# mrmod/h264decode

Measured on AMD Instinct MI355X. Metric: 1080p Main CABAC frames/sec, higher is better.
Workload: dtype u8; 1 GPU; 1920x1080 Main CABAC IPPP GOP-30, 256 independent streams per GPU (32 distinct, each used 8 times), QP 28, 1 slice/frame, 1 ref; parallelism=streams sharded, no collective

## Files before the change

h264decode_amd/csrc/k_entropy.hip:

```cpp
#include <hip/hip_runtime.h>
#include "mi_kernels.h"

#ifndef MI_ENT_ISLICE_PRIO
#define MI_ENT_ISLICE_PRIO 0
#endif
#ifndef MI_ENT_MINWAVES
#define MI_ENT_MINWAVES 6
#endif
#ifndef MI_ENT_B
#define MI_ENT_B 0
#endif
#ifndef MI_ENT_FMO
#define MI_ENT_FMO MI_ENT_B
#endif
#if MI_ENT_B
#define NL 2
#define MI_ENT_KERNEL k_entropy_b
#elif MI_ENT_FMO
#define NL 1
#define MI_ENT_KERNEL k_entropy_f
#else
#define NL 1
#define MI_ENT_KERNEL k_entropy
#endif
#define LANE (e.lane)
#define FI __device__ __forceinline__
#define LDS_SYNC()                                             \
    do {                                                       \
        __builtin_amdgcn_fence(__ATOMIC_RELEASE, "wavefront"); \
        __builtin_amdgcn_wave_barrier();                       \
        __builtin_amdgcn_fence(__ATOMIC_ACQUIRE, "wavefront"); \
    } while (0)

struct TopInfo {
    uint8_t type, t8x8, cbp, chroma_mode, cbf_dc;
    uint8_t dmask;
    uint16_t row;
// ... 728 lines not shown
            off = NB_TL * TB, k = 3;
        else if (gy < 0 && gx == 4)
            off = (NB_TOP + 1) * TB, k = 0, tr = 1;
        const uint32_t interior = gx >= 0 && gx < 4 && gy >= 0;
        return off | k << 9 | edge << 11 | interior << 12 | tr << 13;
    }
    if (l >= 32 && l < 50) {
        const int i = l - 32, cpl = i / 9, g = i % 9, gx = g % 3 - 1, gy = g / 3 - 1;
        uint32_t off = NO_SRC, left = 0;
        if (gy < 0 && gx >= 0)
            off = NB_TOP * TB + static_cast<uint32_t>(offsetof(TopInfo, nnz)) + 4 + cpl * 2 + gx;
        else if (gx < 0 && gy >= 0)
            off = NB_LEFT * TB + static_cast<uint32_t>(offsetof(TopInfo, nnz)) + 4 + cpl * 2 + gy, left = 1;
        const uint32_t interior = gx >= 0 && gy >= 0;
        return off | interior << 12 | left << 14 | static_cast<uint32_t>(cpl * 12 + g) << 16;
    }
    if (l >= 50 && l < 56) {
        const uint32_t left = l < 53;
        return ((left ? NB_LEFT : NB_TOP) * TB + static_cast<uint32_t>(offsetof(TopInfo, cbf_dc))) | static_cast<uint32_t>((l - 50) % 3) << 9 | left << 14;
    }
    return NO_SRC;
}

FI void fill_caches(Ent &e) {
    Shared *s = e.s;
    const bool a_ok = (e.aw & 255) != 0, b_ok = (e.bw & 255) != 0;
    const int cip = e.cip;
    int l = LANE;
    OPAQUE(l);
    const uint32_t role = s->role[l], off = role & NO_SRC;
    const uint8_t *nbb = reinterpret_cast<const uint8_t *>(s->nb);
    int coded = 0;
    if (l < 30) {
        int8_t ipm = -2;
        uint8_t nnz = 0x80;
        const int k = static_cast<int>((role >> 9) & 3u);
        const bool has = off != NO_SRC && !((role >> 13) & 1u && e.mbx + 1 >= e.wmb);
        const TopInfo *n = reinterpret_cast<const TopInfo *>(nbb + (off != NO_SRC ? off : 0u));
        const bool n_ok = has && n->type != MBT_NONE;
        if (n_ok) {
            const int inter = MB_IS_INTER(n->type);
            if (!(cip && inter)) ipm = (n->type == MBT_I4x4 || n->type == MBT_I8x8) ? n->ipm[k] : static_cast<int8_t>(2);
            if ((role >> 11) & 1u) nnz = n->nnz[k];
        }
#pragma unroll
        for (int L = 0; L < NL; L++) {
            int8_t ref = -2, refi = -2;
            uint8_t mvdx = 0, mvdy = 0;
            int16_t mvx = 0, mvy = 0;
            if (n_ok) {
                if (MB_IS_INTER(n->type)) {
                    ref = refi = n->ref[L][k >> 1];
                    mvx = n->mv[L][k][0], mvy = n->mv[L][k][1];
                    mvdx = n->mvd[L][k][0], mvdy = n->mvd[L][k][1];
                    if (MI_ENT_B && ((n->dmask >> (k >> 1)) & 1)) refi = 0;
                } else
                    ref = refi = -1;
            }
            s->ref_c[L][l] = ref;
            s->refi_c[L][l] = refi;
            s->mv_c[L][l][0] = mvx, s->mv_c[L][l][1] = mvy;
            s->mvd_c[L][l][0] = mvdx, s->mvd_c[L][l][1] = mvdy;
        }
        if ((role >> 12) & 1u) {
            nnz = 0;
            ipm = -1;
        }
        coded = (nnz & 0x80) ? 2 : (nnz != 0);
        s->ipm_c[l] = ipm;
        e.v_ipm = ipm;
        s->nnz_c[l] = nnz;
    } else if (l >= 32 && l < 50) {
        const bool ok = off != NO_SRC && (((role >> 14) & 1u) ? a_ok : b_ok);
        const uint8_t v = ((role >> 12) & 1u) ? static_cast<uint8_t>(0) : (ok ? nbb[off != NO_SRC ? off : 0u] : static_cast<uint8_t>(0x80));
        coded = (v & 0x80) ? 2 : (v != 0);
        (&s->nnzc_c[0][0])[(role >> 16) & 31u] = v;
    } else if (l >= 50 && l < 56) {
        const bool ok = ((role >> 14) & 1u) ? a_ok : b_ok;
        coded = ok ? (nbb[off] >> ((role >> 9) & 3u)) & 1 : 2;
    } else if (l >= 56) {
        s->refs8[(l - 56) >> 2][l & 3] = -1;
        if (l < 60) s->sub_type[l - 56] = 0;
        if (l == 60) s->cur_cbf_dc = 0;
    }
    s->coded[l] = static_cast<uint8_t>(coded);
    LDS_SYNC();
}

#if MI_ENT_B
FI int min_positive(int a, int b) { return (a >= 0 && b >= 0) ? min(a, b) : max(a, b); }
FI int b_pair_modes(int k) { return static_cast<int>((0xFB7ED69A5ull >> (4 * k)) & 15); }
FI int b_sub_mode(int st) { return static_cast<int>((0x39FA5E4u >> (2 * st)) & 3); }
FI int b_sub_shape(int st) { return static_cast<int>((0x3F99900u >> (2 * st)) & 3); }
static_assert(((0x39FA5E4u >> 8) & 3) == 1 && ((0x39FA5E4u >> 24) & 3) == 3 && ((0x39FA5E4u >> 12) & 3) == 2 && ((0x3F99900u >> 8) & 3) == 1 && ((0x3F99900u >> 10) & 3) == 2,
              "Table 7-18 constants");

FI void direct_pred(Ent &e, int mask8, bool commit) {
    Shared *s = e.s;
    int l = LANE;
    OPAQUE(l);
    if (l < 20) s->col[l] = e.v_col;
    LDS_SYNC();
    const int bx = l & 3, by = (l >> 2) & 3, q = (by >> 1) * 2 + (bx >> 1);
    const int cb = e.d8inf ? (by >> 1) * 12 + (bx >> 1) * 3 : (l & 15);
// ... 48 lines not shown
        }
        if (!((bx | by) & 1)) {
            if (commit)
                s->refs8[0][q] = static_cast<int8_t>(ref0), s->refs8[1][q] = static_cast<int8_t>(ref1);
            else
                s->dref[0][q] = static_cast<int8_t>(ref0), s->dref[1][q] = static_cast<int8_t>(ref1);
        }
    }
    LDS_SYNC();
}
FI void commit_direct(Ent &e, const int L, int q) {
    Shared *s = e.s;
    const int l = LANE, bx = l & 3, by = (l >> 2) & 3;
    if (l < 16 && (by >> 1) * 2 + (bx >> 1) == q) {
        const int g = GI(bx, by);
        s->ref_c[L][g] = s->dref[L][q];
        *reinterpret_cast<uint32_t *>(s->mv_c[L][g]) = *reinterpret_cast<const uint32_t *>(s->dmv[L][l]);
        if (!((bx | by) & 1)) s->refs8[L][q] = s->dref[L][q];
    }
    LDS_SYNC();
}
#endif

FI void read_ref_idx(Ent &e, const int L, int bx, int by, int w, int h, int nref) {
    Shared *s = e.s;
    int ref = 0;
    if (nref > 1) {
        if (e.cabac) {
            int ctx = (s->refi_c[L][GI(bx - 1, by)] > 0) + 2 * (s->refi_c[L][GI(bx, by - 1)] > 0);
            while (BIN_A(e, 54 + ctx)) {
                ctx = (ctx >> 2) + 4;
                if (++ref > 31) {
                    e.err = 3;
                    break;
                }
            }
        } else
            ref = nref == 2 ? !get_bit(e) : static_cast<int>(get_ue(e));
        if (ref >= nref || ref >= MI_MAX_REFS) e.err = 13, ref = 0;
    }
    {
        const int l = LANE, x = l & 3, y = (l >> 2) & 3;
        if (l < 16 && x >= bx && x < bx + w && y >= by && y < by + h) {
            s->refi_c[L][GI(x, y)] = static_cast<int8_t>(ref);
            if (!((x | y) & 1)) s->refs8[L][(y >> 1) * 2 + (x >> 1)] = static_cast<int8_t>(ref);
        }
        LDS_SYNC();
    }
}
FI void read_mv(Ent &e, const int L, int p) {
    Shared *s = e.s;
    const int bx = p & 3, by = (p >> 2) & 3, w = ((p >> 4) & 3) + 1, h = ((p >> 6) & 3) + 1, shape = (p >> 8) & 7;
    const int ref = s->refs8[L][(by >> 1) * 2 + (bx >> 1)];
    int d[2];
    for (int comp = 0; comp < 2; comp++) {
        int v;
        if (e.cabac) {
            const int sum = s->mvd_c[L][GI(bx - 1, by)][comp] + s->mvd_c[L][GI(bx, by - 1)][comp];
            const int base = comp ? 47 : 40;
            v = 0;
            if (BIN_A(e, base + (sum > 2) + (sum > 32))) {
                int ctx = base + 3;
                v = 1;
                while (v < 9 && BIN_A(e, ctx)) {
                    if (v < 4) ctx++;
                    v++;
                }
                if (v >= 9) v += cabac_egk(e, 3);
                if (cabac_bypass(e)) v = -v;
            }
        } else
            v = get_se(e);
        d[comp] = v;
    }
    int px, py;
    predict_mv(e, L, bx, by, w, ref, shape, px, py);
    set_part(e, L, bx, by, w, h, ref, px + d[0], py + d[1], d[0], d[1]);
}

#if !MI_ENT_B
FI void pskip_fast(Ent &e) {
    Shared *s = e.s;
    int l = LANE;
    OPAQUE(l);
    const uint32_t *nbw = reinterpret_cast<const uint32_t *>(s->nb);
    const uint32_t tA = e.aw, tB = e.bw, tC = nbw[(NB_TOP + 1) * TOP_DW], tD = nbw[NB_TL * TOP_DW];
    const uint32_t rA = nbw[NB_LEFT * TOP_DW + 5], rB = nbw[NB_TOP * TOP_DW + 5], rC = nbw[(NB_TOP + 1) * TOP_DW + 5], rD = nbw[NB_TL * TOP_DW + 5];
    const uint32_t mA = nbw[NB_LEFT * TOP_DW + 6], mB = nbw[NB_TOP * TOP_DW + 6], mC = nbw[(NB_TOP + 1) * TOP_DW + 6], mD = nbw[NB_TL * TOP_DW + 9];
    auto ref_of = [](uint32_t t, uint32_t r, int byte) {
        const int type = static_cast<int>(t & 255u);
        return type == MBT_NONE ? -2 : (MB_IS_INTER(type) ? static_cast<int>(static_cast<int8_t>((r >> (8 * byte)) & 255u)) : -1);
    };
    auto mv_of = [](uint32_t t, uint32_t m) { return MB_IS_INTER(static_cast<int>(t & 255u)) ? m : 0u; };
    const int ra = ref_of(tA, rA, 0), rb = ref_of(tB, rB, 0);
    const bool c_ok = e.mbx + 1 < e.wmb && (tC & 255u) != MBT_NONE;
    const int rc = c_ok ? ref_of(tC, rC, 0) : ref_of(tD, rD, 1);
    const uint32_t va = mv_of(tA, mA), vb = mv_of(tB, mB), vc = c_ok ? mv_of(tC, mC) : mv_of(tD, mD);
    uint32_t mvw = 0;
    const bool zero = ra == -2 || rb == -2 || (ra == 0 && va == 0) || (rb == 0 && vb == 0);
    if (!zero) {
        const int na = ra == 0, nb_ = rb == 0, nc = rc == 0;
        if (na + nb_ + nc == 1)
            mvw = na ? va : (nb_ ? vb : vc);
        else {
            const int ax = static_cast<int16_t>(va & 0xffffu), ay = static_cast<int32_t>(va) >> 16, bx = static_cast<int16_t>(vb & 0xffffu), by = static_cast<int32_t>(vb) >> 16;
            const int cx = static_cast<int16_t>(vc & 0xffffu), cy = static_cast<int32_t>(vc) >> 16;
            mvw = (static_cast<uint32_t>(median3(ax, bx, cx)) & 0xffffu) | (static_cast<uint32_t>(median3(ay, by, cy)) << 16);
        }
    }
    e.cur_type = MBT_PSKIP;
    e.prev_dqp_nz = 0;
    if (l < TOP_DW) {
        const uint32_t row = MI_ENT_FMO ? static_cast<uint32_t>(e.mby + 1) << 16 : 0u;
        const uint32_t nw = l == 0 ? static_cast<uint32_t>(MBT_PSKIP) : (l == 1 ? row : (l == 2 ? 0xFFFFFFFFu : ((l >= 6 && l < 10) ? mvw : 0u)));
        uint32_t *tl = reinterpret_cast<uint32_t *>(&s->nb[NB_TL]), *tp = reinterpret_cast<uint32_t *>(&s->nb[NB_TOP]), *tr = reinterpret_cast<uint32_t *>(&s->nb[NB_TOP + 1]);
        const uint32_t old_top = tp[l], w1 = tr[l];
        tl[l] = old_top;
        tp[l] = w1;
        tr[l] = e.pre_top;
        reinterpret_cast<uint32_t *>(&s->nb[NB_LEFT])[l] = nw;
        reinterpret_cast<uint32_t *>(e.top + e.mbx)[l] = nw;
        e.pre_top = top_load(e, e.mbx + 3, l);
    } else if (l >= 32) {
        const int k = l - 32;
        const uint32_t t = s->skip_tmpl[k];
        const uint32_t w = k == 0 ? (static_cast<uint32_t>(MBT_PSKIP) | e.qpw0) : (k == 1 ? e.qpw1 : ((k >= 12 && k < 28) ? mvw : t));
        const uint64_t mbi = e.mb_base + static_cast<uint64_t>(e.mby) * e.wmb + e.mbx;
        reinterpret_cast<uint32_t *>(e.mbrec + mbi)[k] = w;
    }
    LDS_SYNC();
}
#endif

FI void decode_mb(Ent &e, int skipped) {
    Shared *s = e.s;
    MbRec &r = s->rec;
    const int cabac = e.cabac, islice = e.islice;
    int cbp_luma = 0, cbp_chroma = 0, t8x8 = 0, i16mode = 0, chroma_mode = 0, has_coef = 0;
    int type, raw = 0, nparts = 0;
    const Nb a{e.aw}, b{e.bw};
    r.nzmask = 0;
#if MI_ENT_B
    int no_sub8 = 1;
    e.direct8 = 0;
#endif
    if (skipped) {
#if MI_ENT_B
        type = MBT_BSKIP;
        e.cur_type = type;
        e.direct8 = 15;
        direct_pred(e, 15, true);
#else
        type = MBT_PSKIP;
        e.cur_type = type;
        int mvx = 0, mvy = 0;
        int ra = s->ref_c[0][GI(-1, 0)], rb = s->ref_c[0][GI(0, -1)];
        bool zero = ra == -2 || rb == -2 || (ra == 0 && s->mv_c[0][GI(-1, 0)][0] == 0 && s->mv_c[0][GI(-1, 0)][1] == 0) ||
                    (rb == 0 && s->mv_c[0][GI(0, -1)][0] == 0 && s->mv_c[0][GI(0, -1)][1] == 0);
        if (!zero) predict_mv(e, 0, 0, 0, 4, 0, 0, mvx, mvy);
        set_part(e, 0, 0, 0, 4, 4, 0, mvx, mvy, 0, 0);
        s->refs8[0][0] = s->refs8[0][1] = s->refs8[0][2] = s->refs8[0][3] = 0;
#endif
        e.prev_dqp_nz = 0;
// ... 8 lines not shown
                if (!BIN_A(e, 27 + inc))
                    raw = 0;
                else if (!BIN_A(e, 27 + 3))
                    raw = 1 + BINI_A(e, 27 + 5);
                else {
                    int bits = BINI_A(e, 27 + 4) << 3;
                    bits |= BINI_A(e, 27 + 5) << 2;
                    bits |= BINI_A(e, 27 + 5) << 1;
                    bits |= BINI_A(e, 27 + 5);
                    if (bits < 8)
                        raw = bits + 3;
                    else if (bits == 13)
                        intra_prefix = 1;
                    else if (bits == 14)
                        raw = 11;
                    else if (bits == 15)
                        raw = 22;
                    else
                        raw = ((bits << 1) | BINI_A(e, 27 + 5)) - 4;
                }
            }
#else
            if (!islice) {
                intra_prefix = BINI_A(e, 14);
                if (!intra_prefix) raw = BIN_A(e, 15) ? 2 - BINI_A(e, 17) : 3 * BINI_A(e, 16);
            }
#endif
            if (intra_prefix) {
                int base = islice ? 3 : (MI_ENT_B ? 32 : 17), it = 0, first;
                if (islice) {
                    int inc = (a.ok() && a.type() != MBT_I4x4 && a.type() != MBT_I8x8) + (b.ok() && b.type() != MBT_I4x4 && b.type() != MBT_I8x8);
                    first = BINI_A(e, base + inc);
                    base += 2;
                } else
                    first = BINI_A(e, base);
                if (first) {
                    if (cabac_terminate(e))
                        it = 25;
                    else {
                        it = 1 + 12 * BINI_A(e, base + 1);
                        if (BIN_A(e, base + 2)) it += 4 + 4 * BINI_A(e, base + 2 + islice);
                        it += 2 * BINI_A(e, base + 3 + islice);
                        it += BINI_A(e, base + 3 + 2 * islice);
                    }
                }
                raw = islice ? it : it + (MI_ENT_B ? 23 : 5);
            }
        } else
            raw = static_cast<int>(get_ue(e));
        const int it = islice ? raw : raw - (MI_ENT_B ? 23 : 5);
#if MI_ENT_B
        if (raw < 23)
            type = raw == 0 ? MBT_BDIRECT : MBT_B;
#else
        if (!islice && raw < 5)
            type = raw == 0 ? MBT_P16x16 : (raw == 1 ? MBT_P16x8 : (raw == 2 ? MBT_P8x16 : MBT_P8x8));
#endif
        else if (it == 0)
            type = MBT_I4x4;
        else if (it >= 1 && it <= 24) {
            type = MBT_I16x16;
            i16mode = (it - 1) & 3;
            cbp_chroma = ((it - 1) >> 2) % 3;
            cbp_luma = it >= 13 ? 15 : 0;
            if (cbp_chroma && e.mono) e.err = 25, cbp_chroma = 0;
        } else if (it == 25)
// ... 88 lines not shown
                            int bx, by, w, h, md;
                            if (raw == 22)
                                bx = (i & 1) * 2, by = (i >> 1) * 2, w = 2, h = 2, md = b_sub_mode(s->sub_type[i]);
                            else {
                                const int p = s->parts[i];
                                bx = p & 3, by = (p >> 2) & 3, w = ((p >> 4) & 3) + 1, h = ((p >> 6) & 3) + 1, md = p >> 11;
                            }
                            if ((md >> L) & 1) read_ref_idx(e, L, bx, by, w, h, L ? e.nref1 : e.nref);
                        }
#pragma unroll
                    for (int L = 0; L < 2; L++)
                        for (int i = 0; i < nparts; i++) {
                            const int p = s->parts[i], md = p >> 11;
                            const int bx = p & 3, by = (p >> 2) & 3;
                            if (md == 0)
                                commit_direct(e, L, (by >> 1) * 2 + (bx >> 1));
                            else if ((md >> L) & 1)
                                read_mv(e, L, p);
                            else
                                set_part(e, L, bx, by, ((p >> 4) & 3) + 1, ((p >> 6) & 3) + 1, -1, 0, 0, 0, 0);
                        }
                }
#else
                int nref_parts;
                if (type == MBT_P16x16) {
                    s->parts[0] = PART(0, 0, 4, 4, 0);
                    nparts = nref_parts = 1;
                } else if (type == MBT_P16x8) {
                    s->parts[0] = PART(0, 0, 4, 2, 1), s->parts[1] = PART(0, 2, 4, 2, 2);
                    nparts = nref_parts = 2;
                } else if (type == MBT_P8x16) {
                    s->parts[0] = PART(0, 0, 2, 4, 3), s->parts[1] = PART(2, 0, 2, 4, 4);
                    nparts = nref_parts = 2;
                } else {
                    nref_parts = 4;
                    for (int i = 0; i < 4; i++) {
                        int st;
                        if (cabac)
                            st = BIN_A(e, 21) ? 0 : (!BIN_A(e, 22) ? 1 : (BIN_A(e, 23) ? 2 : 3));
                        else
                            st = static_cast<int>(get_ue(e));
                        if (st > 3) e.err = 21, st = 0;
                        s->sub_type[i] = static_cast<int8_t>(st);
                        const int bx = (i & 1) * 2, by = (i >> 1) * 2;
                        const int sw = (st == 0 || st == 1) ? 2 : 1, sh = (st == 0 || st == 2) ? 2 : 1;
                        for (int yy = 0; yy < 2; yy += sh)
                            for (int xx = 0; xx < 2; xx += sw) s->parts[nparts++] = PART(bx + xx, by + yy, sw, sh, 0);
                    }
                }
                for (int i = 0; i < nref_parts; i++) {
                    int bx, by, w, h;
                    if (type == MBT_P8x8)
                        bx = (i & 1) * 2, by = (i >> 1) * 2, w = 2, h = 2;
                    else {
                        const int p = s->parts[i];
                        bx = p & 3, by = (p >> 2) & 3, w = ((p >> 4) & 3) + 1, h = ((p >> 6) & 3) + 1;
                    }
                    read_ref_idx(e, 0, bx, by, w, h, raw != 4 ? e.nref : 1);
                }
                for (int i = 0; i < nparts; i++) read_mv(e, 0, s->parts[i]);
#endif
            } else {
                if (type == MBT_I4x4 && e.t8x8_mode) {
                    t8x8 = cabac ? BINI_T8(e, (a.ok() && a.t8x8()) + (b.ok() && b.t8x8())) : static_cast<int>(get_bit(e));
                    if (t8x8) type = MBT_I8x8, e.cur_type = type;
                }
                if (type == MBT_I4x4 || type == MBT_I8x8) {
                    const int n = type == MBT_I8x8 ? 4 : 16;
                    for (int i = 0; i < n; i++) {
                        int bx, by;
                        if (n == 4)
                            bx = (i & 1) * 2, by = (i >> 1) * 2;
                        else
                            bx = (i & 1) + 2 * ((i >> 2) & 1), by = ((i >> 1) & 1) + 2 * (i >> 3);
                        const int pa = static_cast<int>(RDL(e.v_ipm, GI(bx - 1, by))), pb = static_cast<int>(RDL(e.v_ipm, GI(bx, by - 1)));
                        const int pred = (pa < -1 || pb < -1) ? 2 : (pa < pb ? pa : pb);
                        int mode = pred;
                        if (cabac) {
                            if (!BIN_B(e, 68)) {
                                int rem = 0;
                                for (int k = 0; k < 3; k++) rem |= BINI_B(e, 69) << k;
                                mode = rem < pred ? rem : rem + 1;
                            }
// ... 8 lines not shown
                }
                if (e.mono)
                    chroma_mode = 0;
                else if (cabac) {
                    int inc = (a.ok() && MB_IS_INTRA(a.type()) && a.type() != MBT_IPCM && a.chroma_mode() != 0) +
                              (b.ok() && MB_IS_INTRA(b.type()) && b.type() != MBT_IPCM && b.chroma_mode() != 0);
                    chroma_mode = 0;
                    if (BIN_B(e, 64 + inc)) {
                        chroma_mode = 1;
                        while (chroma_mode < 3 && BIN_B(e, 67)) chroma_mode++;
                    }
                } else {
                    chroma_mode = static_cast<int>(get_ue(e));
                    if (chroma_mode > 3) e.err = 22, chroma_mode = 0;
                }
                if (LANE < 16) {
                    s->ref_c[0][GI(LANE & 3, LANE >> 2)] = -1;
                    if (MI_ENT_B) s->ref_c[NL - 1][GI(LANE & 3, LANE >> 2)] = -1;
                }
            }
            MI_S(e, MB_IS_INTER(type) ? 1 : 2);
            if (type != MBT_I16x16) {
                int cbp;
                if (cabac) {
                    const int cbp_a = a.ok() ? (a.type() == MBT_IPCM ? 0x2F : a.cbp()) : 0x0F;
                    const int cbp_b = b.ok() ? (b.type() == MBT_IPCM ? 0x2F : b.cbp()) : 0x0F;
                    cbp = 0;
                    for (int b8 = 0; b8 < 4; b8++) {
                        int ca = (b8 & 1) ? (cbp >> (b8 - 1)) & 1 : (cbp_a >> (b8 + 1)) & 1;
                        int cb = (b8 & 2) ? (cbp >> (b8 - 2)) & 1 : (cbp_b >> (b8 + 2)) & 1;
                        cbp |= BINI_B(e, 73 + (!ca) + 2 * (!cb)) << b8;
                    }
                    int ca = a.ok() && (a.type() == MBT_IPCM || (a.cbp() >> 4) != 0), cb = b.ok() && (b.type() == MBT_IPCM || (b.cbp() >> 4) != 0);
                    if (!e.mono && BIN_B(e, 77 + ca + 2 * cb)) {
                        ca = a.ok() && (a.type() == MBT_IPCM || (a.cbp() >> 4) == 2);
                        cb = b.ok() && (b.type() == MBT_IPCM || (b.cbp() >> 4) == 2);
                        cbp |= (1 + BINI_B(e, 77 + 4 + ca + 2 * cb)) << 4;
                    }
                } else {
                    uint32_t k = get_ue(e);
                    if (k > (e.mono ? 15u : 47u)) e.err = 23, k = 0;
                    if (e.mono) k += 48;
                    cbp = RFL(static_cast<int>(MB_IS_INTRA(type) ? e.tab->me_intra[k] : e.tab->me_inter[k]));
                }
                cbp_luma = cbp & 15, cbp_chroma = cbp >> 4;
                if (cbp_luma && e.t8x8_mode && MB_IS_INTER(type)) {
#if MI_ENT_B
                    const int all8 = no_sub8;
#else
                    int all8 = 1;
                    if (type == MBT_P8x8)
                        for (int i = 0; i < 4; i++) all8 &= s->sub_type[i] == 0;
#endif
                    if (all8) t8x8 = cabac ? BINI_T8(e, (a.ok() && a.t8x8()) + (b.ok() && b.t8x8())) : static_cast<int>(get_bit(e));
                }
            }
            if (cbp_luma || cbp_chroma || type == MBT_I16x16) {
                int dqp;
                if (cabac) {
                    int ctx = e.prev_dqp_nz ? 1 : 0, val = 0;
                    while (BIN_A(e, 60 + ctx)) {
                        ctx = 2 + (ctx >> 1);
// ... 93 lines not shown
    TopInfo *tp = &s->nb[NB_TOP];
    if (l >= 32 && l < 32 + TOP_DW) reinterpret_cast<uint32_t *>(&s->nb[NB_TL])[l - 32] = reinterpret_cast<const uint32_t *>(tp)[l - 32];
    LDS_SYNC();
    if (l < 2) {
        TopInfo *dst = &s->nb[l == 0 ? NB_TOP : NB_LEFT];
        dst->type = static_cast<uint8_t>(type);
        dst->t8x8 = static_cast<uint8_t>(t8x8);
        dst->cbp = r.cbp;
        dst->chroma_mode = static_cast<uint8_t>(chroma_mode);
        dst->cbf_dc = s->cur_cbf_dc;
        if (MI_ENT_FMO) dst->row = static_cast<uint16_t>(e.mby + 1);
#pragma unroll
        for (int L = 0; L < NL; L++) {
            dst->ref[L][0] = inter ? s->refs8[L][l == 0 ? 2 : 1] : static_cast<int8_t>(-1);
            dst->ref[L][1] = inter ? s->refs8[L][3] : static_cast<int8_t>(-1);
        }
#if MI_ENT_B
        dst->dmask = static_cast<uint8_t>(l == 0 ? (e.direct8 >> 2) & 3 : ((e.direct8 >> 1) & 1) | ((e.direct8 >> 2) & 2));
#endif
    } else if (l >= 8 && l < 16) {
        int k = l & 3, is_left = l >= 12;
        TopInfo *dst = &s->nb[is_left ? NB_LEFT : NB_TOP];
        int g = is_left ? GI(3, k) : GI(k, 3);
        dst->ipm[k] = s->ipm_c[g];
        dst->nnz[k] = s->nnz_c[g];
#pragma unroll
        for (int L = 0; L < NL; L++) {
            dst->mv[L][k][0] = s->mv_c[L][g][0], dst->mv[L][k][1] = s->mv_c[L][g][1];
            dst->mvd[L][k][0] = s->mvd_c[L][g][0], dst->mvd[L][k][1] = s->mvd_c[L][g][1];
        }
    } else if (l >= 16 && l < 24) {
        int i = l - 16, is_left = i >= 4, cpl = (i >> 1) & 1, k = i & 1;
        TopInfo *dst = &s->nb[is_left ? NB_LEFT : NB_TOP];
        dst->nnz[4 + cpl * 2 + k] = is_left ? s->nnzc_c[cpl][(k + 1) * 3 + 2] : s->nnzc_c[cpl][2 * 3 + k + 1];
    }
    LDS_SYNC();
    if (l < TOP_DW) {
        const uint32_t nw = reinterpret_cast<const uint32_t *>(tp)[l], w1 = reinterpret_cast<const uint32_t *>(&s->nb[NB_TOP + 1])[l];
        reinterpret_cast<uint32_t *>(e.top + e.mbx)[l] = nw;
        reinterpret_cast<uint32_t *>(&s->nb[NB_TOP])[l] = w1;
        reinterpret_cast<uint32_t *>(&s->nb[NB_TOP + 1])[l] = e.pre_top;
        e.pre_top = top_load(e, e.mbx + 3, l);
    }
    const uint64_t mbi = e.mb_base + static_cast<uint64_t>(e.mby) * e.wmb + e.mbx;
    if (l >= 32)
        reinterpret_cast<uint32_t *>(e.mbrec + mbi)[l - 32] = reinterpret_cast<const uint32_t *>(&r)[l - 32];
#if MI_ENT_B
// ... 138 lines not shown
    int addr = RFL(static_cast<int>(sd->first_mb));
    const bool fmo = MI_ENT_FMO && RFL(static_cast<int>(pd->fmo)) != 0;
    bool consecutive = false;
    if (!fmo) fill_none(e, RFL(static_cast<int>(sd->fill_from)), min(addr, total));
    e.mbx = addr % e.wmb, e.mby = addr / e.wmb;
    int more = 1, skip_state = 0 , pending = 0;
    int n_mbs = 0;
    while (more && !e.err) {
        if (addr >= total) {
            e.err = 30;
            break;
        }
        if (fmo) {
            asm volatile("s_waitcnt vmcnt(0)" ::: "memory");
            if (!consecutive && l < TOP_DW) {
                reinterpret_cast<uint32_t *>(&sh.nb[NB_LEFT])[l] = 0;
                reinterpret_cast<uint32_t *>(&sh.nb[NB_TL])[l] = e.mbx > 0 ? top_load(e, e.mbx - 1, l) : 0u;
            }
            if (l < 2 * TOP_DW) reinterpret_cast<uint32_t *>(&sh.nb[NB_TOP])[l] = top_load(e, e.mbx + l / TOP_DW, l % TOP_DW);
            LDS_SYNC();
            if (l < 3 && sh.nb[NB_TL + l].row != static_cast<uint16_t>(e.mby)) sh.nb[NB_TL + l].type = MBT_NONE;
            LDS_SYNC();
        } else if (e.mbx == 0 || n_mbs == 0) {
            if (l < TOP_DW) reinterpret_cast<uint32_t *>(&sh.nb[NB_LEFT])[l] = 0, reinterpret_cast<uint32_t *>(&sh.nb[NB_TL])[l] = 0;
            asm volatile("s_waitcnt vmcnt(0)" ::: "memory");
            if (l < 2 * TOP_DW) reinterpret_cast<uint32_t *>(&sh.nb[NB_TOP])[l] = top_load(e, e.mbx + l / TOP_DW, l % TOP_DW);
            if (l < TOP_DW) e.pre_top = top_load(e, e.mbx + 2, l);
            LDS_SYNC();
        }
        OPAQUE(e.lane);
        slide_window(e);
        MI_T0(e);
#if MI_ENT_B
        e.v_col = (e.col && l < 20) ? e.col[static_cast<size_t>(addr) * 20 + l] : ((l >= 16 && l < 19) ? 0xFFFFFFFFu : 0u);
#endif
        e.aw = RFL(*reinterpret_cast<const uint32_t *>(&sh.nb[NB_LEFT])), e.bw = RFL(*reinterpret_cast<const uint32_t *>(&sh.nb[NB_TOP]));
        int skipped = 0;
        if (!e.islice) {
            if (e.cabac) {
                const Nb a{e.aw}, b{e.bw};
                const int skip_type = MI_ENT_B ? MBT_BSKIP : MBT_PSKIP;
                skipped = BINI_A(e, (MI_ENT_B ? 24 : 11) + (a.ok() && a.type() != skip_type) + (b.ok() && b.type() != skip_type));
            } else {
                if (skip_state == 0) {
                    pending = static_cast<int>(get_ue(e));
                    if (pending > total - addr) e.err = 31, pending = 0;
                    if (pending > 0) skip_state = 1;
                }
                if (skip_state == 1) {
                    skipped = 1;
                    pending--;
                }
            }
        }
#if !MI_ENT_B
        if (skipped) {
            MI_T(e, 1);
            pskip_fast(e);
        } else
#endif
        {
            MI_T(e, 1);
            fill_caches(e);
            MI_T(e, 0);
            decode_mb(e, skipped);
        }
        MI_T(e, 3);
        if (e.err) break;
        n_mbs++;
        if (e.cabac)
            more = !cabac_terminate(e);
        else if (skipped) {
            if (pending == 0) {
                more = bitpos(e) < stop_bit;
                skip_state = 2;
            }
        } else {
            more = bitpos(e) < stop_bit;
            skip_state = 0;
        }
        if (fmo) {
            const uint8_t *sgmap = bitstream + RFL(e.pd->sgmap_off);
            const int sgroup = RFL(static_cast<int>(sgmap[RFL(static_cast<int>(e.sd->first_mb))]));
            const uint32_t inv_wmb = RFL(e.pd->inv_wmb);
            int next = total;
            for (int base = addr + 1; base < total; base += 64) {
                const int i = base + l;
                const unsigned long long m = __builtin_amdgcn_ballot_w64(i < total && sgmap[i] == sgroup);
                if (m) {
// ... 27 lines not shown
```

Before: 29380 frames/s.

## Add fast path for CABAC P16x16 macroblocks in entropy kernel

For non-B CABAC P slices, the mb_type prefix is now decoded before the neighbour caches are filled. P16x16 macroblocks decode ref_idx, mvd and cbp straight from packed neighbour words. A P16x16 with zero cbp leaves through a shared skip-style writer, which skips fill_caches and the general partition loops. A coded P16x16 runs a reduced fill_caches that omits ipm and per-block ref/mv setup. This is meant to cut LDS traffic and wave barriers per inter macroblock, at the cost of more code paths that must stay bit-exact.

```diff
diff --git a/h264decode_amd/csrc/k_entropy.hip b/h264decode_amd/csrc/k_entropy.hip
--- a/h264decode_amd/csrc/k_entropy.hip
+++ b/h264decode_amd/csrc/k_entropy.hip
@@ -13,6 +13,10 @@
 #ifndef MI_ENT_FMO
 #define MI_ENT_FMO MI_ENT_B
 #endif
+#ifndef MI_ENT_P16_DIRECT
+#define MI_ENT_P16_DIRECT 1
+#endif
+#define MI_P16 (MI_ENT_P16_DIRECT && !MI_ENT_B)
 #if MI_ENT_B
 #define NL 2
 #define MI_ENT_KERNEL k_entropy_b
@@ -787,7 +791,7 @@
     return NO_SRC;
 }
 
-FI void fill_caches(Ent &e) {
+FI void fill_caches(Ent &e, bool p16 = false, uint32_t mvw = 0, uint32_t mvdw = 0, int ref16 = 0) {
     Shared *s = e.s;
     const bool a_ok = (e.aw & 255) != 0, b_ok = (e.bw & 255) != 0;
     const int cip = e.cip;
@@ -797,43 +801,44 @@
     const uint8_t *nbb = reinterpret_cast<const uint8_t *>(s->nb);
     int coded = 0;
     if (l < 30) {
-        int8_t ipm = -2;
         uint8_t nnz = 0x80;
         const int k = static_cast<int>((role >> 9) & 3u);
         const bool has = off != NO_SRC && !((role >> 13) & 1u && e.mbx + 1 >= e.wmb);
         const TopInfo *n = reinterpret_cast<const TopInfo *>(nbb + (off != NO_SRC ? off : 0u));
         const bool n_ok = has && n->type != MBT_NONE;
-        if (n_ok) {
-            const int inter = MB_IS_INTER(n->type);
-            if (!(cip && inter)) ipm = (n->type == MBT_I4x4 || n->type == MBT_I8x8) ? n->ipm[k] : static_cast<int8_t>(2);
-            if ((role >> 11) & 1u) nnz = n->nnz[k];
-        }
+        const bool interior = (role >> 12) & 1u;
+        if (n_ok && ((role >> 11) & 1u)) nnz = n->nnz[k];
+        if (interior) nnz = 0;
+        if (!p16) {
+            int8_t ipm = -2;
+            if (n_ok && !(cip && MB_IS_INTER(n->type))) ipm = (n->type == MBT_I4x4 || n->type == MBT_I8x8) ? n->ipm[k] : static_cast<int8_t>(2);
+            if (interior) ipm = -1;
+            s->ipm_c[l] = ipm;
+            e.v_ipm = ipm;
 #pragma unroll
-        for (int L = 0; L < NL; L++) {
-            int8_t ref = -2, refi = -2;
-            uint8_t mvdx = 0, mvdy = 0;
-            int16_t mvx = 0, mvy = 0;
-            if (n_ok) {
-                if (MB_IS_INTER(n->type)) {
-                    ref = refi = n->ref[L][k >> 1];
-                    mvx = n->mv[L][k][0], mvy = n->mv[L][k][1];
-                    mvdx = n->mvd[L][k][0], mvdy = n->mvd[L][k][1];
-                    if (MI_ENT_B && ((n->dmask >> (k >> 1)) & 1)) refi = 0;
-                } else
-                    ref = refi = -1;
+            for (int L = 0; L < NL; L++) {
+                int8_t ref = -2, refi = -2;
+                uint8_t mvdx = 0, mvdy = 0;
+                int16_t mvx = 0, mvy = 0;
+                if (n_ok) {
+                    if (MB_IS_INTER(n->type)) {
+                        ref = refi = n->ref[L][k >> 1];
+                        mvx = n->mv[L][k][0], mvy = n->mv[L][k][1];
+                        mvdx = n->mvd[L][k][0], mvdy = n->mvd[L][k][1];
+                        if (MI_ENT_B && ((n->dmask >> (k >> 1)) & 1)) refi = 0;
+                    } else
+                        ref = refi = -1;
+                }
+                s->ref_c[L][l] = ref;
+                s->refi_c[L][l] = refi;
+                s->mv_c[L][l][0] = mvx, s->mv_c[L][l][1] = mvy;
+                s->mvd_c[L][l][0] = mvdx, s->mvd_c[L][l][1] = mvdy;
             }
-            s->ref_c[L][l] = ref;
-            s->refi_c[L][l] = refi;
-            s->mv_c[L][l][0] = mvx, s->mv_c[L][l][1] = mvy;
-            s->mvd_c[L][l][0] = mvdx, s->mvd_c[L][l][1] = mvdy;
-        }
-        if ((role >> 12) & 1u) {
-            nnz = 0;
-            ipm = -1;
+        } else if (interior) {
+            *reinterpret_cast<uint32_t *>(s->mv_c[0][l]) = mvw;
+            *reinterpret_cast<uint16_t *>(s->mvd_c[0][l]) = static_cast<uint16_t>(mvdw);
         }
         coded = (nnz & 0x80) ? 2 : (nnz != 0);
-        s->ipm_c[l] = ipm;
-        e.v_ipm = ipm;
         s->nnz_c[l] = nnz;
     } else if (l >= 32 && l < 50) {
         const bool ok = off != NO_SRC && (((role >> 14) & 1u) ? a_ok : b_ok);
@@ -844,7 +849,7 @@
         const bool ok = ((role >> 14) & 1u) ? a_ok : b_ok;
         coded = ok ? (nbb[off] >> ((role >> 9) & 3u)) & 1 : 2;
     } else if (l >= 56) {
-        s->refs8[(l - 56) >> 2][l & 3] = -1;
+        s->refs8[(l - 56) >> 2][l & 3] = static_cast<int8_t>((p16 && l < 60) ? ref16 : -1);
         if (l < 60) s->sub_type[l - 56] = 0;
         if (l == 60) s->cur_cbf_dc = 0;
     }
@@ -939,20 +944,57 @@
 }
 #endif
 
+FI int cabac_ref_idx(Ent &e, int ctx) {
+    int ref = 0;
+    while (BIN_A(e, 54 + ctx)) {
+        ctx = (ctx >> 2) + 4;
+        if (++ref > 31) {
+            e.err = 3;
+            break;
+        }
+    }
+    return ref;
+}
+FI int cabac_mvd(Ent &e, int comp, int sum) {
+    const int base = comp ? 47 : 40;
+    int v = 0;
+    if (BIN_A(e, base + (sum > 2) + (sum > 32))) {
+        int ctx = base + 3;
+        v = 1;
+        while (v < 9 && BIN_A(e, ctx)) {
+            if (v < 4) ctx++;
+            v++;
+        }
+        if (v >= 9) v += cabac_egk(e, 3);
+        if (cabac_bypass(e)) v = -v;
+    }
+    return v;
+}
+FI int cabac_cbp(Ent &e, const Nb a, const Nb b) {
+    const int cbp_a = a.ok() ? (a.type() == MBT_IPCM ? 0x2F : a.cbp()) : 0x0F;
+    const int cbp_b = b.ok() ? (b.type() == MBT_IPCM ? 0x2F : b.cbp()) : 0x0F;
+    int cbp = 0;
+    for (int b8 = 0; b8 < 4; b8++) {
+        int ca = (b8 & 1) ? (cbp >> (b8 - 1)) & 1 : (cbp_a >> (b8 + 1)) & 1;
+        int cb = (b8 & 2) ? (cbp >> (b8 - 2)) & 1 : (cbp_b >> (b8 + 2)) & 1;
+        cbp |= BINI_B(e, 73 + (!ca) + 2 * (!cb)) << b8;
+    }
+    int ca = a.ok() && (a.type() == MBT_IPCM || (a.cbp() >> 4) != 0), cb = b.ok() && (b.type() == MBT_IPCM || (b.cbp() >> 4) != 0);
+    if (!e.mono && BIN_B(e, 77 + ca + 2 * cb)) {
+        ca = a.ok() && (a.type() == MBT_IPCM || (a.cbp() >> 4) == 2);
+        cb = b.ok() && (b.type() == MBT_IPCM || (b.cbp() >> 4) == 2);
+        cbp |= (1 + BINI_B(e, 77 + 4 + ca + 2 * cb)) << 4;
+    }
+    return cbp;
+}
+
 FI void read_ref_idx(Ent &e, const int L, int bx, int by, int w, int h, int nref) {
     Shared *s = e.s;
     int ref = 0;
     if (nref > 1) {
-        if (e.cabac) {
-            int ctx = (s->refi_c[L][GI(bx - 1, by)] > 0) + 2 * (s->refi_c[L][GI(bx, by - 1)] > 0);
-            while (BIN_A(e, 54 + ctx)) {
-                ctx = (ctx >> 2) + 4;
-                if (++ref > 31) {
-                    e.err = 3;
-                    break;
-                }
-            }
-        } else
+        if (e.cabac)
+            ref = cabac_ref_idx(e, (s->refi_c[L][GI(bx - 1, by)] > 0) + 2 * (s->refi_c[L][GI(bx, by - 1)] > 0));
+        else
             ref = nref == 2 ? !get_bit(e) : static_cast<int>(get_ue(e));
         if (ref >= nref || ref >= MI_MAX_REFS) e.err = 13, ref = 0;
     }
@@ -972,21 +1014,9 @@
     int d[2];
     for (int comp = 0; comp < 2; comp++) {
         int v;
-        if (e.cabac) {
-            const int sum = s->mvd_c[L][GI(bx - 1, by)][comp] + s->mvd_c[L][GI(bx, by - 1)][comp];
-            const int base = comp ? 47 : 40;
-            v = 0;
-            if (BIN_A(e, base + (sum > 2) + (sum > 32))) {
-                int ctx = base + 3;
-                v = 1;
-                while (v < 9 && BIN_A(e, ctx)) {
-                    if (v < 4) ctx++;
-                    v++;
-                }
-                if (v >= 9) v += cabac_egk(e, 3);
-                if (cabac_bypass(e)) v = -v;
-            }
-        } else
+        if (e.cabac)
+            v = cabac_mvd(e, comp, s->mvd_c[L][GI(bx - 1, by)][comp] + s->mvd_c[L][GI(bx, by - 1)][comp]);
+        else
             v = get_se(e);
         d[comp] = v;
     }
@@ -996,40 +1026,43 @@
 }
 
 #if !MI_ENT_B
-FI void pskip_fast(Ent &e) {
+FI int nb_ref(uint32_t t, uint32_t r, int byte) {
+    const int type = static_cast<int>(t & 255u);
+    return type == MBT_NONE ? -2 : (MB_IS_INTER(type) ? static_cast<int>(static_cast<int8_t>((r >> (8 * byte)) & 255u)) : -1);
+}
+FI uint32_t nb_mv(uint32_t t, uint32_t m) { return MB_IS_INTER(static_cast<int>(t & 255u)) ? m : 0u; }
+struct Nb3 {
+    int ra, rb, rc;
+    uint32_t va, vb, vc;
+};
+FI Nb3 nb_abc(const Ent &e) {
+    const uint32_t *nbw = reinterpret_cast<const uint32_t *>(e.s->nb);
+    const uint32_t tA = e.aw, tB = e.bw, tC = nbw[(NB_TOP + 1) * TOP_DW], tD = nbw[NB_TL * TOP_DW];
+    const uint32_t rA = nbw[NB_LEFT * TOP_DW + 5], rB = nbw[NB_TOP * TOP_DW + 5], rC = nbw[(NB_TOP + 1) * TOP_DW + 5], rD = nbw[NB_TL * TOP_DW + 5];
+    const uint32_t mA = nbw[NB_LEFT * TOP_DW + 6], mB = nbw[NB_TOP * TOP_DW + 6], mC = nbw[(NB_TOP + 1) * TOP_DW + 6], mD = nbw[NB_TL * TOP_DW + 9];
+    const bool c_ok = e.mbx + 1 < e.wmb && (tC & 255u) != MBT_NONE;
+    Nb3 n;
+    n.ra = nb_ref(tA, rA, 0), n.rb = nb_ref(tB, rB, 0), n.rc = c_ok ? nb_ref(tC, rC, 0) : nb_ref(tD, rD, 1);
+    n.va = nb_mv(tA, mA), n.vb = nb_mv(tB, mB), n.vc = c_ok ? nb_mv(tC, mC) : nb_mv(tD, mD);
+    return n;
+}
+FI uint32_t nb_predict(int ra, int rb, int rc, uint32_t va, uint32_t vb, uint32_t vc, int ref) {
+    const int na = ra == ref, nb_ = rb == ref, nc = rc == ref;
+    if (na + nb_ + nc == 1) return na ? va : (nb_ ? vb : vc);
+    const int ax = static_cast<int16_t>(va & 0xffffu), ay = static_cast<int32_t>(va) >> 16, bx = static_cast<int16_t>(vb & 0xffffu), by = static_cast<int32_t>(vb) >> 16;
+    const int cx = static_cast<int16_t>(vc & 0xffffu), cy = static_cast<int32_t>(vc) >> 16;
+    return (static_cast<uint32_t>(median3(ax, bx, cx)) & 0xffffu) | (static_cast<uint32_t>(median3(ay, by, cy)) << 16);
+}
+FI void p_leave(Ent &e, int type, uint32_t mvw, uint32_t mvdw, int ref) {
     Shared *s = e.s;
     int l = LANE;
     OPAQUE(l);
-    const uint32_t *nbw = reinterpret_cast<const uint32_t *>(s->nb);
-    const uint32_t tA = e.aw, tB = e.bw, tC = nbw[(NB_TOP + 1) * TOP_DW], tD = nbw[NB_TL * TOP_DW];
-    const uint32_t rA = nbw[NB_LEFT * TOP_DW + 5], rB = nbw[NB_TOP * TOP_DW + 5], rC = nbw[(NB_TOP + 1) * TOP_DW + 5], rD = nbw[NB_TL * TOP_DW + 5];
-    const uint32_t mA = nbw[NB_LEFT * TOP_DW + 6], mB = nbw[NB_TOP * TOP_DW + 6], mC = nbw[(NB_TOP + 1) * TOP_DW + 6], mD = nbw[NB_TL * TOP_DW + 9];
-    auto ref_of = [](uint32_t t, uint32_t r, int byte) {
-        const int type = static_cast<int>(t & 255u);
-        return type == MBT_NONE ? -2 : (MB_IS_INTER(type) ? static_cast<int>(static_cast<int8_t>((r >> (8 * byte)) & 255u)) : -1);
-    };
-    auto mv_of = [](uint32_t t, uint32_t m) { return MB_IS_INTER(static_cast<int>(t & 255u)) ? m : 0u; };
-    const int ra = ref_of(tA, rA, 0), rb = ref_of(tB, rB, 0);
-    const bool c_ok = e.mbx + 1 < e.wmb && (tC & 255u) != MBT_NONE;
-    const int rc = c_ok ? ref_of(tC, rC, 0) : ref_of(tD, rD, 1);
-    const uint32_t va = mv_of(tA, mA), vb = mv_of(tB, mB), vc = c_ok ? mv_of(tC, mC) : mv_of(tD, mD);
-    uint32_t mvw = 0;
-    const bool zero = ra == -2 || rb == -2 || (ra == 0 && va == 0) || (rb == 0 && vb == 0);
-    if (!zero) {
-        const int na = ra == 0, nb_ = rb == 0, nc = rc == 0;
-        if (na + nb_ + nc == 1)
-            mvw = na ? va : (nb_ ? vb : vc);
-        else {
-            const int ax = static_cast<int16_t>(va & 0xffffu), ay = static_cast<int32_t>(va) >> 16, bx = static_cast<int16_t>(vb & 0xffffu), by = static_cast<int32_t>(vb) >> 16;
-            const int cx = static_cast<int16_t>(vc & 0xffffu), cy = static_cast<int32_t>(vc) >> 16;
-            mvw = (static_cast<uint32_t>(median3(ax, bx, cx)) & 0xffffu) | (static_cast<uint32_t>(median3(ay, by, cy)) << 16);
-        }
-    }
-    e.cur_type = MBT_PSKIP;
+    e.cur_type = type;
     e.prev_dqp_nz = 0;
     if (l < TOP_DW) {
         const uint32_t row = MI_ENT_FMO ? static_cast<uint32_t>(e.mby + 1) << 16 : 0u;
-        const uint32_t nw = l == 0 ? static_cast<uint32_t>(MBT_PSKIP) : (l == 1 ? row : (l == 2 ? 0xFFFFFFFFu : ((l >= 6 && l < 10) ? mvw : 0u)));
+        uint32_t nw = l == 0 ? static_cast<uint32_t>(type) : (l == 1 ? row : (l == 2 ? 0xFFFFFFFFu : ((l >= 6 && l < 10) ? mvw : 0u)));
+        if (MI_P16) nw = l == 5 ? static_cast<uint32_t>(ref) * 0x0101u : (l >= 10 ? mvdw * 0x00010001u : nw);
         uint32_t *tl = reinterpret_cast<uint32_t *>(&s->nb[NB_TL]), *tp = reinterpret_cast<uint32_t *>(&s->nb[NB_TOP]), *tr = reinterpret_cast<uint32_t *>(&s->nb[NB_TOP + 1]);
         const uint32_t old_top = tp[l], w1 = tr[l];
         tl[l] = old_top;
@@ -1041,21 +1074,63 @@
     } else if (l >= 32) {
         const int k = l - 32;
         const uint32_t t = s->skip_tmpl[k];
-        const uint32_t w = k == 0 ? (static_cast<uint32_t>(MBT_PSKIP) | e.qpw0) : (k == 1 ? e.qpw1 : ((k >= 12 && k < 28) ? mvw : t));
+        uint32_t w = k == 0 ? (static_cast<uint32_t>(type) | e.qpw0) : (k == 1 ? e.qpw1 : ((k >= 12 && k < 28) ? mvw : t));
+        if (MI_P16) {
+            const uint32_t slot = RFL(static_cast<uint32_t>(static_cast<uint16_t>(s->ref_slot[0][ref & (MI_MAX_REFS - 1)])));
+            w = k == 8 ? static_cast<uint32_t>(ref) * 0x01010101u : ((k == 9 || k == 10) ? slot * 0x00010001u : w);
+        }
         const uint64_t mbi = e.mb_base + static_cast<uint64_t>(e.mby) * e.wmb + e.mbx;
         reinterpret_cast<uint32_t *>(e.mbrec + mbi)[k] = w;
     }
     LDS_SYNC();
 }
-#endif
-
-FI void decode_mb(Ent &e, int skipped) {
+FI uint32_t pskip_vector(const Ent &e) {
+    const Nb3 n = nb_abc(e);
+    const bool zero = n.ra == -2 || n.rb == -2 || (n.ra == 0 && n.va == 0) || (n.rb == 0 && n.vb == 0);
+    return zero ? 0u : nb_predict(n.ra, n.rb, n.rc, n.va, n.vb, n.vc, 0);
+}
+FI int p16_syntax(Ent &e, uint32_t &mvw, uint32_t &mvdw, int &ref) {
+    const uint32_t *nbw = reinterpret_cast<const uint32_t *>(e.s->nb);
+    ref = 0;
+    if (e.nref > 1) {
+        const int ra = nb_ref(e.aw, nbw[NB_LEFT * TOP_DW + 5], 0), rb = nb_ref(e.bw, nbw[NB_TOP * TOP_DW + 5], 0);
+        ref = cabac_ref_idx(e, RFL((ra > 0) + 2 * (rb > 0)));
+        if (ref >= e.nref || ref >= MI_MAX_REFS) e.err = 13, ref = 0;
+    }
+    const uint32_t dA = nb_mv(e.aw, nbw[NB_LEFT * TOP_DW + 10]), dB = nb_mv(e.bw, nbw[NB_TOP * TOP_DW + 10]);
+    const uint32_t sums = RFL(((dA & 255u) + (dB & 255u)) | (((dA >> 8) & 255u) + ((dB >> 8) & 255u)) << 16);
+    int dx = 0, dy = 0;
+#pragma unroll 1
+    for (int comp = 0; comp < 2; comp++) {
+        const int v = cabac_mvd(e, comp, static_cast<int>((sums >> (16 * comp)) & 0xffffu));
+        dx = comp ? dx : v, dy = comp ? v : dy;
+    }
+    const Nb3 n = nb_abc(e);
+    const bool only_a = n.rb == -2 && n.rc == -2 && n.ra != -2;
+    const uint32_t pw = nb_predict(n.ra, only_a ? n.ra : n.rb, only_a ? n.ra : n.rc, n.va, only_a ? n.va : n.vb, only_a ? n.va : n.vc, ref);
+    mvw = RFL(((pw + static_cast<uint32_t>(dx)) & 0xffffu) | ((pw >> 16) + static_cast<uint32_t>(dy)) << 16);
+    mvdw = static_cast<uint32_t>(min(abs(dx), 255) | min(abs(dy), 255) << 8);
+    MI_S(e, 1);
+    const int cbp = cabac_cbp(e, Nb{e.aw}, Nb{e.bw});
+    MI_S(e, 2);
+    return cbp;
+}
+#endif
+
+FI int mb_type_prefix(Ent &e, int &raw) {
+    const int intra_prefix = BINI_A(e, 14);
+    if (!intra_prefix) raw = BIN_A(e, 15) ? 2 - BINI_A(e, 17) : 3 * BINI_A(e, 16);
+    return intra_prefix;
+}
+enum { PRE_INTRA = 8, PRE_P16 = 16 };
+FI void decode_mb(Ent &e, int skipped, int pre = -1) {
     Shared *s = e.s;
     MbRec &r = s->rec;
     const int cabac = e.cabac, islice = e.islice;
     int cbp_luma = 0, cbp_chroma = 0, t8x8 = 0, i16mode = 0, chroma_mode = 0, has_coef = 0;
     int type, raw = 0, nparts = 0;
     const Nb a{e.aw}, b{e.bw};
+    const bool p16 = MI_P16 && pre >= PRE_P16;
     r.nzmask = 0;
 #if MI_ENT_B
     int no_sub8 = 1;
@@ -1110,12 +1185,16 @@
             }
 #else
             if (!islice) {
-                intra_prefix = BINI_A(e, 14);
-                if (!intra_prefix) raw = BIN_A(e, 15) ? 2 - BINI_A(e, 17) : 3 * BINI_A(e, 16);
+#if MI_P16
+                intra_prefix = pre == PRE_INTRA, raw = p16 ? 0 : pre & 3;
+#else
+                intra_prefix = mb_type_prefix(e, raw);
+#endif
             }
 #endif
             if (intra_prefix) {
                 int base = islice ? 3 : (MI_ENT_B ? 32 : 17), it = 0, first;
+                const int isl = RFL(islice);
                 if (islice) {
                     int inc = (a.ok() && a.type() != MBT_I4x4 && a.type() != MBT_I8x8) + (b.ok() && b.type() != MBT_I4x4 && b.type() != MBT_I8x8);
                     first = BINI_A(e, base + inc);
@@ -1127,9 +1206,9 @@
                         it = 25;
                     else {
                         it = 1 + 12 * BINI_A(e, base + 1);
-                        if (BIN_A(e, base + 2)) it += 4 + 4 * BINI_A(e, base + 2 + islice);
-                        it += 2 * BINI_A(e, base + 3 + islice);
-                        it += BINI_A(e, base + 3 + 2 * islice);
+                        if (BIN_A(e, base + 2)) it += 4 + 4 * BINI_A(e, base + 2 + isl);
+                        it += 2 * BINI_A(e, base + 3 + isl);
+                        it += BINI_A(e, base + 3 + 2 * isl);
                     }
                 }
                 raw = islice ? it : it + (MI_ENT_B ? 23 : 5);
@@ -1264,43 +1343,45 @@
                         }
                 }
 #else
-                int nref_parts;
-                if (type == MBT_P16x16) {
-                    s->parts[0] = PART(0, 0, 4, 4, 0);
-                    nparts = nref_parts = 1;
-                } else if (type == MBT_P16x8) {
-                    s->parts[0] = PART(0, 0, 4, 2, 1), s->parts[1] = PART(0, 2, 4, 2, 2);
-                    nparts = nref_parts = 2;
-                } else if (type == MBT_P8x16) {
-                    s->parts[0] = PART(0, 0, 2, 4, 3), s->parts[1] = PART(2, 0, 2, 4, 4);
-                    nparts = nref_parts = 2;
-                } else {
-                    nref_parts = 4;
-                    for (int i = 0; i < 4; i++) {
-                        int st;
-                        if (cabac)
-                            st = BIN_A(e, 21) ? 0 : (!BIN_A(e, 22) ? 1 : (BIN_A(e, 23) ? 2 : 3));
-                        else
-                            st = static_cast<int>(get_ue(e));
-                        if (st > 3) e.err = 21, st = 0;
-                        s->sub_type[i] = static_cast<int8_t>(st);
-                        const int bx = (i & 1) * 2, by = (i >> 1) * 2;
-                        const int sw = (st == 0 || st == 1) ? 2 : 1, sh = (st == 0 || st == 2) ? 2 : 1;
-                        for (int yy = 0; yy < 2; yy += sh)
-                            for (int xx = 0; xx < 2; xx += sw) s->parts[nparts++] = PART(bx + xx, by + yy, sw, sh, 0);
+                if (!p16) {
+                    int nref_parts;
+                    if (type == MBT_P16x16) {
+                        s->parts[0] = PART(0, 0, 4, 4, 0);
+                        nparts = nref_parts = 1;
+                    } else if (type == MBT_P16x8) {
+                        s->parts[0] = PART(0, 0, 4, 2, 1), s->parts[1] = PART(0, 2, 4, 2, 2);
+                        nparts = nref_parts = 2;
+                    } else if (type == MBT_P8x16) {
+                        s->parts[0] = PART(0, 0, 2, 4, 3), s->parts[1] = PART(2, 0, 2, 4, 4);
+                        nparts = nref_parts = 2;
+                    } else {
+                        nref_parts = 4;
+                        for (int i = 0; i < 4; i++) {
+                            int st;
+                            if (cabac)
+                                st = BIN_A(e, 21) ? 0 : (!BIN_A(e, 22) ? 1 : (BIN_A(e, 23) ? 2 : 3));
+                            else
+                                st = static_cast<int>(get_ue(e));
+                            if (st > 3) e.err = 21, st = 0;
+                            s->sub_type[i] = static_cast<int8_t>(st);
+                            const int bx = (i & 1) * 2, by = (i >> 1) * 2;
+                            const int sw = (st == 0 || st == 1) ? 2 : 1, sh = (st == 0 || st == 2) ? 2 : 1;
+                            for (int yy = 0; yy < 2; yy += sh)
+                                for (int xx = 0; xx < 2; xx += sw) s->parts[nparts++] = PART(bx + xx, by + yy, sw, sh, 0);
+                        }
                     }
+                    for (int i = 0; i < nref_parts; i++) {
+                        int bx, by, w, h;
+                        if (type == MBT_P8x8)
+                            bx = (i & 1) * 2, by = (i >> 1) * 2, w = 2, h = 2;
+                        else {
+                            const int p = s->parts[i];
+                            bx = p & 3, by = (p >> 2) & 3, w = ((p >> 4) & 3) + 1, h = ((p >> 6) & 3) + 1;
+                        }
+                        read_ref_idx(e, 0, bx, by, w, h, raw != 4 ? e.nref : 1);
+                    }
+                    for (int i = 0; i < nparts; i++) read_mv(e, 0, s->parts[i]);
                 }
-                for (int i = 0; i < nref_parts; i++) {
-                    int bx, by, w, h;
-                    if (type == MBT_P8x8)
-                        bx = (i & 1) * 2, by = (i >> 1) * 2, w = 2, h = 2;
-                    else {
-                        const int p = s->parts[i];
-                        bx = p & 3, by = (p >> 2) & 3, w = ((p >> 4) & 3) + 1, h = ((p >> 6) & 3) + 1;
-                    }
-                    read_ref_idx(e, 0, bx, by, w, h, raw != 4 ? e.nref : 1);
-                }
-                for (int i = 0; i < nparts; i++) read_mv(e, 0, s->parts[i]);
 #endif
             } else {
                 if (type == MBT_I4x4 && e.t8x8_mode) {
@@ -1355,22 +1436,11 @@
             MI_S(e, MB_IS_INTER(type) ? 1 : 2);
             if (type != MBT_I16x16) {
                 int cbp;
-                if (cabac) {
-                    const int cbp_a = a.ok() ? (a.type() == MBT_IPCM ? 0x2F : a.cbp()) : 0x0F;
-                    const int cbp_b = b.ok() ? (b.type() == MBT_IPCM ? 0x2F : b.cbp()) : 0x0F;
-                    cbp = 0;
-                    for (int b8 = 0; b8 < 4; b8++) {
-                        int ca = (b8 & 1) ? (cbp >> (b8 - 1)) & 1 : (cbp_a >> (b8 + 1)) & 1;
-                        int cb = (b8 & 2) ? (cbp >> (b8 - 2)) & 1 : (cbp_b >> (b8 + 2)) & 1;
-                        cbp |= BINI_B(e, 73 + (!ca) + 2 * (!cb)) << b8;
-                    }
-                    int ca = a.ok() && (a.type() == MBT_IPCM || (a.cbp() >> 4) != 0), cb = b.ok() && (b.type() == MBT_IPCM || (b.cbp() >> 4) != 0);
-                    if (!e.mono && BIN_B(e, 77 + ca + 2 * cb)) {
-                        ca = a.ok() && (a.type() == MBT_IPCM || (a.cbp() >> 4) == 2);
-                        cb = b.ok() && (b.type() == MBT_IPCM || (b.cbp() >> 4) == 2);
-                        cbp |= (1 + BINI_B(e, 77 + 4 + ca + 2 * cb)) << 4;
-                    }
-                } else {
+                if (p16)
+                    cbp = pre - PRE_P16;
+                else if (cabac)
+                    cbp = cabac_cbp(e, a, b);
+                else {
                     uint32_t k = get_ue(e);
                     if (k > (e.mono ? 15u : 47u)) e.err = 23, k = 0;
                     if (e.mono) k += 48;
@@ -1510,7 +1580,7 @@
         int k = l & 3, is_left = l >= 12;
         TopInfo *dst = &s->nb[is_left ? NB_LEFT : NB_TOP];
         int g = is_left ? GI(3, k) : GI(k, 3);
-        dst->ipm[k] = s->ipm_c[g];
+        dst->ipm[k] = (MI_P16 && inter) ? static_cast<int8_t>(-1) : s->ipm_c[g];
         dst->nnz[k] = s->nnz_c[g];
 #pragma unroll
         for (int L = 0; L < NL; L++) {
@@ -1695,10 +1765,12 @@
             if (l < 3 && sh.nb[NB_TL + l].row != static_cast<uint16_t>(e.mby)) sh.nb[NB_TL + l].type = MBT_NONE;
             LDS_SYNC();
         } else if (e.mbx == 0 || n_mbs == 0) {
-            if (l < TOP_DW) reinterpret_cast<uint32_t *>(&sh.nb[NB_LEFT])[l] = 0, reinterpret_cast<uint32_t *>(&sh.nb[NB_TL])[l] = 0;
+            int lr = LANE;
+            OPAQUE(lr);
+            if (lr < TOP_DW) reinterpret_cast<uint32_t *>(&sh.nb[NB_LEFT])[lr] = 0, reinterpret_cast<uint32_t *>(&sh.nb[NB_TL])[lr] = 0;
             asm volatile("s_waitcnt vmcnt(0)" ::: "memory");
-            if (l < 2 * TOP_DW) reinterpret_cast<uint32_t *>(&sh.nb[NB_TOP])[l] = top_load(e, e.mbx + l / TOP_DW, l % TOP_DW);
-            if (l < TOP_DW) e.pre_top = top_load(e, e.mbx + 2, l);
+            if (lr < 2 * TOP_DW) reinterpret_cast<uint32_t *>(&sh.nb[NB_TOP])[lr] = top_load(e, e.mbx + lr / TOP_DW, lr % TOP_DW);
+            if (lr < TOP_DW) e.pre_top = top_load(e, e.mbx + 2, lr);
             LDS_SYNC();
         }
         OPAQUE(e.lane);
@@ -1726,18 +1798,32 @@
                 }
             }
         }
-#if !MI_ENT_B
-        if (skipped) {
-            MI_T(e, 1);
-            pskip_fast(e);
-        } else
-#endif
-        {
-            MI_T(e, 1);
-            fill_caches(e);
+#if MI_ENT_B
+        MI_T(e, 1);
+        fill_caches(e);
+        MI_T(e, 0);
+        decode_mb(e, skipped);
+#else
+        int pre = -1, ref = 0;
+        uint32_t mvw = 0, mvdw = 0;
+        if (skipped)
+            mvw = pskip_vector(e);
+        else if (MI_P16 && !e.islice && e.cabac) {
+            int raw = 0;
+            MI_S(e, 3);
+            pre = mb_type_prefix(e, raw) ? PRE_INTRA : raw;
+            MI_S(e, 0);
+            if (pre == 0) pre = PRE_P16 + p16_syntax(e, mvw, mvdw, ref);
+        }
+        MI_T(e, 1);
+        if (skipped || pre == PRE_P16)
+            p_leave(e, skipped ? MBT_PSKIP : MBT_P16x16, mvw, mvdw, ref);
+        else {
+            fill_caches(e, MI_P16 && pre > PRE_P16, mvw, mvdw, ref);
             MI_T(e, 0);
-            decode_mb(e, skipped);
-        }
+            decode_mb(e, 0, pre);
+        }
+#endif
         MI_T(e, 3);
         if (e.err) break;
         n_mbs++;
```

Result: no change. 29630 frames/s (median of 6 runs) (+0.8%).
